# MPEGGroup/mpeg-pcc-tmc2

Measured on AMD Instinct MI355X. Metric: encoder patch+image-gen frames/sec, longdress_vox10 32-frame GOF, higher is better.
Workload: dtype int32/f64

## Files before the change

mpeg-pcc-tmc2_amd/csrc/kdtree_device.hip:

```cpp
#include <algorithm>
#include <cstring>

#include "internal.h"
#include "wave.h"

namespace tmc2 {
namespace {

constexpr uint32_t kNone      = 0xFFFFFFFFu;
constexpr int      kBlock     = 256;
constexpr int      kWaves     = kBlock / 64;
constexpr int      kScanTile  = kBlock * 8;
constexpr int      kLeafMax   = 10;
constexpr int      kMaxLevels = 64;

struct BuildSeg {
  uint32_t begin, end;
  uint32_t node, parent;
  int32_t  mn[3], mx[3];
  int16_t  lo[3], hi[3];
  uint8_t  side, pdim;
  uint8_t  split, cutDim;
  int32_t  cut;
  uint32_t mid;
  uint32_t slot;
};

struct RetiredSeg {
  uint32_t begin, end, node, level;
  int16_t  lo[3], hi[3];
  int32_t  root;
};

struct HugeSeg {
  uint32_t begin, end, node, level;
  int16_t  lo[3], hi[3];
  int32_t  root;
  int32_t  mn[3], mx[3];
};

struct BuildArgs {
  const Pt* pts;
  uint32_t  n, tiles;
  Pt*       P;
  uint32_t *perm, *seg;
  BuildSeg *segA, *segB;
  KdNode*   nodes;
  uint32_t *loc1, *loc2, *tile1, *tile2;
  uint32_t* counts;
  uint32_t* nodeCount;
  int32_t*  rootBox;
  uint32_t* levels;
  RetiredSeg* retired;
  uint32_t*   retiredCount;
  uint32_t*   bigCount;
  HugeSeg*    huge;
  uint32_t*   hugeCount;
  uint32_t    hugeMax;
  uint32_t    retireMax, splitMax;
  struct LvSeg *lvA, *lvB;
  uint16_t*   list;
  struct LvPartial* partial;
  unsigned long long* pieceProfile;
  uint32_t    decideRng;
  uint32_t*   finishDepth;
  uint32_t*   ticket;
  volatile uint32_t* hostSmall;
  volatile uint32_t* hostDepth;
};

__device__ __forceinline__ int coordOf( const Pt p, int d ) { return d == 0 ? p.x : ( d == 1 ? p.y : p.z ); }

struct SplitRule {
  int     dim;
  int32_t cut;
};
__device__ __forceinline__ SplitRule splitOf( const int16_t ( &lo )[3], const int16_t ( &hi )[3], const int32_t ( &mn )[3],
                                              const int32_t ( &mx )[3] ) {
  const int32_t maxSpan = max( int32_t( hi[0] ) - lo[0], max( int32_t( hi[1] ) - lo[1], int32_t( hi[2] ) - lo[2] ) );
  SplitRule     r;
  r.dim              = 0;
  int32_t bestSpread = -1;
#pragma unroll
  for ( int d = 0; d < 3; ++d ) {
    if ( double( int32_t( hi[d] ) - lo[d] ) > ( 1.0 - 0.00001 ) * double( maxSpan ) ) {
      const int32_t spread = mx[d] - mn[d];
      if ( spread > bestSpread ) {
        bestSpread = spread;
        r.dim      = d;
      }
    }
  }
  const int32_t l = r.dim == 0 ? lo[0] : ( r.dim == 1 ? lo[1] : lo[2] ), h = r.dim == 0 ? hi[0] : ( r.dim == 1 ? hi[1] : hi[2] );
  const int32_t a = r.dim == 0 ? mn[0] : ( r.dim == 1 ? mn[1] : mn[2] ), b = r.dim == 0 ? mx[0] : ( r.dim == 1 ? mx[1] : mx[2] );
  r.cut           = min( max( ( l + h ) / 2, a ), b );
  return r;
}

constexpr int      kHugeWaves = 16;
constexpr uint32_t kHugeLimit = 131072;
constexpr int      kHugeNodes = 2 * int( kHugeLimit / 4096 ) + 4;
struct HugeNode {
  uint32_t begin, end;
  uint32_t node;
  int16_t  lo[3], hi[3];
  int16_t  mn[3], mx[3];
  uint16_t depth;
};

__device__ __forceinline__ uint32_t blockClassLists( const Pt* pts, uint32_t count, int dim, int32_t c, uint32_t* listGE,
                                                     uint32_t* listLT, uint32_t* waveCnt ) {
  const int lane = threadIdx.x & 63, wave = threadIdx.x >> 6;
  uint32_t  mGE = 0, mIn = 0;
  int       buf = 0;
  for ( uint32_t base = 0; base < count; base += 4u * blockDim.x, buf ^= 1 ) {
    const uint32_t i0 = base + 4u * threadIdx.x;
    bool           ge[4];
    uint32_t       cGE = 0, cIn = 0;
#pragma unroll
    for ( int j = 0; j < 4; ++j ) {
      const bool    in = i0 + j < count;
      const int32_t x  = coordOf( pts[in ? i0 + j : 0u], dim );
      ge[j]            = in && x >= c;
      cGE += uint32_t( ge[j] ), cIn += uint32_t( in );
    }
    const uint32_t inc = waveInclusive( cGE | ( cIn << 16 ), lane );
    if ( lane == 63 ) waveCnt[buf * kHugeWaves + wave] = inc;
    __syncthreads();
    uint32_t before = 0, total = 0;
#pragma unroll
    for ( int w = 0; w < kHugeWaves; ++w ) {
      const uint32_t cw = waveCnt[buf * kHugeWaves + w];
      total += cw;
      before += w < wave ? cw : 0u;
    }
    before += inc - ( cGE | ( cIn << 16 ) );
    uint32_t atGE = mGE + ( before & 0xFFFFu ) + 0u, atIn = mIn + ( before >> 16 );
#pragma unroll
    for ( int j = 0; j < 4; ++j ) {
      if ( i0 + j < count ) {
        if ( ge[j] )
          listGE[atGE] = i0 + j;
        else
          listLT[atIn - atGE] = i0 + j;
        atGE += uint32_t( ge[j] ), ++atIn;
      }
    }
    mGE += total & 0xFFFFu, mIn += total >> 16;
  }
  return mGE;
}

__device__ __forceinline__ uint32_t blockSweep( Pt* pts, uint32_t* id, uint32_t count, int dim, int32_t c, uint32_t* listGE,
                                                uint32_t* listLT, uint32_t* waveCnt ) {
  const uint32_t nGE = blockClassLists( pts, count, dim, c, listGE, listLT, waveCnt ), nL = count - nGE;
  __syncthreads();
  for ( uint32_t t = threadIdx.x; t < min( nGE, nL ); t += blockDim.x ) {
    const uint32_t x = listGE[t];
    if ( x >= nL ) break;
    const uint32_t y  = listLT[nL - 1u - t];
    const Pt       px = pts[x], py = pts[y];
    const uint32_t ix = id[x], iy = id[y];
    pts[x] = py, pts[y] = px, id[x] = iy, id[y] = ix;
  }
  __syncthreads();
  return nL;
}

__global__ __launch_bounds__( 64 * kHugeWaves ) void hugeSegmentsKernel( BuildArgs a ) {
  __shared__ HugeNode sNode[2][kHugeNodes];
  __shared__ uint32_t sCount[2], waveCnt[2 * kHugeWaves];
  __shared__ int32_t  red[kHugeWaves][12];
  const int      lane = threadIdx.x & 63, wave = threadIdx.x >> 6;
  const uint32_t total = *a.hugeCount;
  for ( uint32_t s = blockIdx.x; s < total; s += gridDim.x ) {
    const HugeSeg seg = a.huge[s];
    __syncthreads();
    if ( threadIdx.x == 0 ) {
      HugeNode r;
      r.begin = 0, r.end = seg.end - seg.begin, r.node = seg.node, r.depth = 0;
      for ( int d = 0; d < 3; ++d ) r.lo[d] = seg.lo[d], r.hi[d] = seg.hi[d], r.mn[d] = int16_t( seg.mn[d] ), r.mx[d] = int16_t( seg.mx[d] );
      sNode[0][0] = r;
      sCount[0] = 1, sCount[1] = 0;
    }
    __syncthreads();
    int cur = 0;
    for ( uint32_t depth = 0;; ++depth ) {
      const uint32_t nCur = sCount[cur];
      if ( nCur == 0 ) break;
      for ( uint32_t t = 0; t < nCur; ++t ) {
        const HugeNode q     = sNode[cur][t];
        const uint32_t count = q.end - q.begin;
        if ( uint32_t( q.depth ) + seg.level >= uint32_t( kMaxLevels ) - 2u ) {
          if ( threadIdx.x == 0 ) atomicMax( a.finishDepth, 0x10000u );
          continue;
        }
        Pt*       pts = a.P + seg.begin + q.begin;
        uint32_t* id  = a.perm + seg.begin + q.begin;
        int32_t   mn[3], mx[3];
        const bool isRoot = seg.root != 0 && depth == 0;
        int16_t    lo[3], hi[3];
        for ( int d = 0; d < 3; ++d ) mn[d] = q.mn[d], mx[d] = q.mx[d], lo[d] = isRoot ? q.mn[d] : q.lo[d], hi[d] = isRoot ? q.mx[d] : q.hi[d];
        const SplitRule rule  = splitOf( lo, hi, mn, mx );
        uint32_t*       listA = a.loc1 + seg.begin + q.begin;
        uint32_t*       listB = a.loc2 + seg.begin + q.begin;
        const uint32_t  lt    = blockSweep( pts, id, count, rule.dim, rule.cut, listA, listB, waveCnt );
        const uint32_t  le    = lt + blockSweep( pts + lt, id + lt, count - lt, rule.dim, rule.cut + 1, listA, listB, waveCnt );
        const uint32_t  half  = count / 2;
        const uint32_t  idx   = lt > half ? lt : ( le < half ? le : half );
        int32_t r[12];
#pragma unroll
        for ( int k = 0; k < 12; ++k ) r[k] = ( k % 6 ) < 3 ? 0x7FFFFFFF : int32_t( 0x80000000 );
        for ( uint32_t base = 0; base < count; base += 4u * blockDim.x ) {
          Pt p[4];
#pragma unroll
          for ( int j = 0; j < 4; ++j ) {
            const uint32_t i = base + j * blockDim.x + threadIdx.x;
            p[j]             = pts[i < count ? i : 0u];
          }
#pragma unroll
          for ( int j = 0; j < 4; ++j ) {
            const uint32_t i = base + j * blockDim.x + threadIdx.x;
            if ( i < count ) {
              const int o = i < idx ? 0 : 6;
              if ( o == 0 ) {
                r[0] = min( r[0], int32_t( p[j].x ) ), r[1] = min( r[1], int32_t( p[j].y ) ), r[2] = min( r[2], int32_t( p[j].z ) );
                r[3] = max( r[3], int32_t( p[j].x ) ), r[4] = max( r[4], int32_t( p[j].y ) ), r[5] = max( r[5], int32_t( p[j].z ) );
              } else {
                r[6] = min( r[6], int32_t( p[j].x ) ), r[7] = min( r[7], int32_t( p[j].y ) ), r[8] = min( r[8], int32_t( p[j].z ) );
                r[9] = max( r[9], int32_t( p[j].x ) ), r[10] = max( r[10], int32_t( p[j].y ) ), r[11] = max( r[11], int32_t( p[j].z ) );
              }
            }
          }
        }
#pragma unroll
        for ( int off = 32; off > 0; off >>= 1 )
#pragma unroll
          for ( int k = 0; k < 12; ++k ) {
            const int32_t o = __shfl_xor( r[k], off, 64 );
            r[k]            = ( k % 6 ) < 3 ? min( r[k], o ) : max( r[k], o );
          }
        if ( lane == 0 )
          for ( int k = 0; k < 12; ++k ) red[wave][k] = r[k];
        __syncthreads();
        if ( threadIdx.x == 0 ) {
          for ( int w = 0; w < kHugeWaves; ++w )
            for ( int k = 0; k < 12; ++k ) r[k] = ( k % 6 ) < 3 ? min( r[k], red[w][k] ) : max( r[k], red[w][k] );
          const uint32_t id0 = atomicAdd( a.nodeCount, 2u );
          KdNode         nd;
          nd.a = int32_t( id0 ), nd.b = int32_t( id0 + 1 ), nd.divlow = int16_t( r[3 + rule.dim] ), nd.divhigh = int16_t( r[6 + rule.dim] ),
          nd.dim = rule.dim;
          a.nodes[q.node] = nd;
          HugeNode child[2];
          child[0].begin = q.begin, child[0].end = q.begin + idx, child[0].node = id0;
          child[1].begin = q.begin + idx, child[1].end = q.end, child[1].node = id0 + 1;
          for ( int c = 0; c < 2; ++c ) {
            child[c].depth = uint16_t( q.depth + 1 );
            for ( int d = 0; d < 3; ++d )
              child[c].lo[d] = lo[d], child[c].hi[d] = hi[d], child[c].mn[d] = int16_t( r[6 * c + d] ), child[c].mx[d] = int16_t( r[6 * c + 3 + d] );
          }
          const int16_t cut = int16_t( rule.cut );
          if ( rule.dim == 0 ) child[0].hi[0] = cut, child[1].lo[0] = cut;
          if ( rule.dim == 1 ) child[0].hi[1] = cut, child[1].lo[1] = cut;
          if ( rule.dim == 2 ) child[0].hi[2] = cut, child[1].lo[2] = cut;
          for ( int c = 0; c < 2; ++c ) {
            const uint32_t cc = child[c].end - child[c].begin, level = seg.level + child[c].depth;
            if ( cc <= uint32_t( kLeafMax ) ) {
              KdNode leaf;
              leaf.a = int32_t( seg.begin + child[c].begin ), leaf.b = int32_t( seg.begin + child[c].end ), leaf.divlow = leaf.divhigh = 0,
              leaf.dim = -1;
              a.nodes[child[c].node] = leaf;
              atomicMax( a.finishDepth, level + 1u );
            } else if ( cc <= a.retireMax ) {
              RetiredSeg rs;
              rs.begin = seg.begin + child[c].begin, rs.end = seg.begin + child[c].end, rs.node = child[c].node, rs.level = level, rs.root = 0;
              for ( int d = 0; d < 3; ++d ) rs.lo[d] = child[c].lo[d], rs.hi[d] = child[c].hi[d];
              a.retired[atomicAdd( a.retiredCount, 1u )] = rs;
            } else {
              sNode[cur ^ 1][sCount[cur ^ 1]++] = child[c];
            }
          }
        }
        __syncthreads();
      }
      if ( threadIdx.x == 0 ) sCount[cur] = 0;
      cur ^= 1;
      __syncthreads();
    }
  }
}

constexpr int      kPieceMax  = 4096;
constexpr int      kPieceRecs = kPieceMax / ( kLeafMax + 1 ) + 2;
constexpr uint16_t kNoRec     = 0xFFFFu;
constexpr uint32_t kNoKey     = 0xFFFFFFFFu;

struct alignas( 8 ) PieceRec {
  uint16_t begin, end;
  int16_t  cut;
  uint8_t  dim, unused0;
// ... 15 lines not shown
  uint32_t e1rb1, e2rb2;
};
struct PieceHot2 {
  uint32_t midc0, c1;
};

__device__ __forceinline__ void pieceBarrier() { asm volatile( "s_waitcnt lgkmcnt(0)\n\ts_barrier" ::: "memory" ); }

typedef short pkShort2 __attribute__( ( ext_vector_type( 2 ) ) );
__device__ __forceinline__ uint32_t pkMin( uint32_t a, uint32_t b ) {
  return __builtin_bit_cast( uint32_t, __builtin_elementwise_min( __builtin_bit_cast( pkShort2, a ), __builtin_bit_cast( pkShort2, b ) ) );
}
__device__ __forceinline__ uint32_t pkMax( uint32_t a, uint32_t b ) {
  return __builtin_bit_cast( uint32_t, __builtin_elementwise_max( __builtin_bit_cast( pkShort2, a ), __builtin_bit_cast( pkShort2, b ) ) );
}
__device__ __forceinline__ uint32_t pk2( int lo16, int hi16 ) { return ( uint32_t( lo16 ) & 0xFFFFu ) | ( uint32_t( hi16 ) << 16 ); }
__device__ __forceinline__ int      pkLo( uint32_t v ) { return int( int16_t( v & 0xFFFFu ) ); }
__device__ __forceinline__ int      pkHi( uint32_t v ) { return int( int16_t( v >> 16 ) ); }

template <int WAVES>
__device__ __forceinline__ uint32_t pieceScan( uint32_t v, uint32_t* waveTot ) {
  const int lane = threadIdx.x & 63, wave = threadIdx.x >> 6;
  const uint32_t inc = waveInclusive( v, lane );
  if ( lane == 63 ) waveTot[wave] = inc;
  pieceBarrier();
  uint32_t before = 0;
#pragma unroll
  for ( int w = 0; w < WAVES; w += 4 ) {
    const uint4 t = *reinterpret_cast<const uint4*>( waveTot + w );
    before += ( w + 0 < wave ? t.x : 0u ) + ( w + 1 < wave ? t.y : 0u ) + ( w + 2 < wave ? t.z : 0u ) + ( w + 3 < wave ? t.w : 0u );
  }
  return before + inc - v;
}

__device__ __forceinline__ bool waveSegMinMaxPacked( uint32_t key, uint32_t& A, uint32_t& B, uint32_t& C, int lane ) {
#pragma unroll
  for ( int off = 1; off < 64; off <<= 1 ) {
    const uint32_t ok = __shfl_down( key, off, 64 );
    const uint32_t oa = __shfl_down( A, off, 64 ), ob = __shfl_down( B, off, 64 ), oc = __shfl_down( C, off, 64 );
    if ( lane + off < 64 && ok == key ) A = pkMin( A, oa ), B = pkMax( B, ob ), C = pkMin( C, oc );
  }
  const uint32_t pk = __shfl_up( key, 1, 64 );
  return key != kNoKey && ( lane == 0 || pk != key );
}

__device__ __forceinline__ void ldsMin( int32_t* slot, int32_t v ) {
  if ( v < *reinterpret_cast<volatile int32_t*>( slot ) ) atomicMin( slot, v );
}
__device__ __forceinline__ void ldsMax( int32_t* slot, int32_t v ) {
  if ( v > *reinterpret_cast<volatile int32_t*>( slot ) ) atomicMax( slot, v );
}


struct LvSeg {
  uint32_t begin, end;
  uint32_t cutInfo;
  uint32_t edge1;
  uint32_t slot;
  uint32_t childNode;
  uint32_t node, parent;
  int16_t  lo[3], hi[3];
  uint8_t  side, pdim;
  uint16_t unused;
  int32_t  mn[3], mx[3];
};

constexpr int kLandBlock = 256;
constexpr int kLandRounds = 2;
struct LvPartial {
  uint32_t slot;
  uint32_t v[6];
  uint32_t unused;
};

__device__ __forceinline__ void lvReport( LvSeg* child, int mnx, int mny, int mnz, int mxx, int mxy, int mxz ) {
  if ( mnx < loadStaleOk( &child->mn[0] ) ) atomicMin( &child->mn[0], mnx );
  if ( mny < loadStaleOk( &child->mn[1] ) ) atomicMin( &child->mn[1], mny );
  if ( mnz < loadStaleOk( &child->mn[2] ) ) atomicMin( &child->mn[2], mnz );
  if ( mxx > loadStaleOk( &child->mx[0] ) ) atomicMax( &child->mx[0], mxx );
  if ( mxy > loadStaleOk( &child->mx[1] ) ) atomicMax( &child->mx[1], mxy );
  if ( mxz > loadStaleOk( &child->mx[2] ) ) atomicMax( &child->mx[2], mxz );
}

__device__ __forceinline__ uint32_t lvPrefix( const uint32_t* __restrict__ loc, const uint32_t* sums, uint32_t tiles, uint32_t i, uint32_t n ) {
  return i < n ? loc[i] + sums[i / kScanTile] : sums[tiles];
}

__device__ __forceinline__ uint32_t lvPartner( const uint16_t* __restrict__ list, const uint32_t* sums, uint32_t from, uint32_t to, uint32_t G ) {
  uint32_t lo = from / kScanTile, hi = ( to - 1u ) / kScanTile;
  while ( lo < hi ) {
    const uint32_t mid = ( lo + hi + 1u ) / 2u;
    if ( mid * kScanTile - sums[mid] <= G )
      lo = mid;
    else
      hi = mid - 1u;
  }
  return lo * kScanTile + list[size_t( lo ) * kScanTile + ( G - ( lo * kScanTile - sums[lo] ) )];
}

__global__ __launch_bounds__( kBlock ) void lvInitKernel( BuildArgs a ) {
  __shared__ int blockRange[6 * kWaves];
  const uint32_t n = a.n, gsize = gridDim.x * blockDim.x;
  const int      lane = threadIdx.x & 63, wave = threadIdx.x >> 6;
  int mnx = 0x7FFFFFFF, mny = mnx, mnz = mnx, mxx = int( 0x80000000 ), mxy = mxx, mxz = mxx;
  for ( uint32_t i = blockIdx.x * blockDim.x + threadIdx.x; i < n; i += gsize ) {
    const Pt p = a.pts[i];
    a.P[i]     = p;
    a.perm[i]  = i;
    a.seg[i]   = 0;
    mnx = min( mnx, int( p.x ) ), mny = min( mny, int( p.y ) ), mnz = min( mnz, int( p.z ) );
    mxx = max( mxx, int( p.x ) ), mxy = max( mxy, int( p.y ) ), mxz = max( mxz, int( p.z ) );
  }
  mnx = waveMin( mnx ), mny = waveMin( mny ), mnz = waveMin( mnz );
  mxx = waveMax( mxx ), mxy = waveMax( mxy ), mxz = waveMax( mxz );
  if ( lane == 0 ) {
    int* w = blockRange + 6 * wave;
    w[0] = mnx, w[1] = mny, w[2] = mnz, w[3] = mxx, w[4] = mxy, w[5] = mxz;
  }
  __syncthreads();
  if ( threadIdx.x < 6 ) {
    int v = blockRange[threadIdx.x];
    for ( int w = 1; w < kWaves; ++w ) v = threadIdx.x < 3 ? min( v, blockRange[6 * w + threadIdx.x] ) : max( v, blockRange[6 * w + threadIdx.x] );
    int32_t* slot = threadIdx.x < 3 ? &a.lvA[0].mn[threadIdx.x] : &a.lvA[0].mx[threadIdx.x - 3];
    if ( threadIdx.x < 3 ) {
      if ( v < loadStaleOk( slot ) ) atomicMin( slot, v );
    } else {
      if ( v > loadStaleOk( slot ) ) atomicMax( slot, v );
    }
  }
}
__global__ void lvRootKernel( BuildArgs a ) {
  if ( threadIdx.x < kMaxLevels + 16 ) a.counts[threadIdx.x] = 0;
  __syncthreads();
  if ( threadIdx.x != 0 ) return;
  LvSeg r{};
  r.begin = 0, r.end = a.n, r.node = 0, r.parent = kNone;
  for ( int d = 0; d < 3; ++d ) r.mn[d] = 0x7FFFFFFF, r.mx[d] = int32_t( 0x80000000 );
  a.lvA[0]     = r;
// ... 85 lines not shown
        const int32_t maxSpan = max( hi[0] - lo[0], max( hi[1] - lo[1], hi[2] - lo[2] ) );
        const double  limit   = ( 1.0 - 0.00001 ) * double( maxSpan );
        int           dim     = 0;
        int32_t       best    = -1;
        if ( double( hi[0] - lo[0] ) > limit && mx[0] - mn[0] > best ) best = mx[0] - mn[0], dim = 0;
        if ( double( hi[1] - lo[1] ) > limit && mx[1] - mn[1] > best ) best = mx[1] - mn[1], dim = 1;
        if ( double( hi[2] - lo[2] ) > limit && mx[2] - mn[2] > best ) best = mx[2] - mn[2], dim = 2;
        const int32_t l = dim == 0 ? lo[0] : ( dim == 1 ? lo[1] : lo[2] ), h = dim == 0 ? hi[0] : ( dim == 1 ? hi[1] : hi[2] );
        const int32_t lowest = dim == 0 ? mn[0] : ( dim == 1 ? mn[1] : mn[2] ), highest = dim == 0 ? mx[0] : ( dim == 1 ? mx[1] : mx[2] );
        const int32_t cut = min( max( ( l + h ) / 2, lowest ), highest );
        q->cutInfo = ( uint32_t( cut ) & 0xFFFFu ) | ( uint32_t( dim ) << 16 ) | ( 1u << 24 );
        if ( root )
          for ( int d = 0; d < 3; ++d ) q->lo[d] = int16_t( mn[d] ), q->hi[d] = int16_t( mx[d] );
        split = 1;
      }
      if ( !split ) q->cutInfo = 0;
    }
    const uint32_t inc = waveInclusive( split, lane );
    if ( lane == 63 ) waveTot[wave] = inc;
    __syncthreads();
    uint32_t before = sCarry, all = 0;
    for ( int w = 0; w < kDecideThreads / 64; ++w ) {
      all += waveTot[w];
      before += w < wave ? waveTot[w] : 0u;
    }
    const uint32_t rank = before + inc - split;
    if ( split ) q->slot = 2u * rank, q->childNode = nodeBase + 2u * rank;
    __syncthreads();
    if ( threadIdx.x == 0 ) sCarry += all;
    __syncthreads();
  }
  if ( threadIdx.x == 0 ) {
    a.counts[level + 1] = 2u * sCarry;
    *a.nodeCount        = nodeBase + 2u * sCarry;
  }
  if ( a.hostSmall ) {
    if ( threadIdx.x == 0 ) __threadfence();
    __syncthreads();
    if ( threadIdx.x < kMaxLevels + 16 ) a.hostSmall[threadIdx.x] = __hip_atomic_load( &a.counts[threadIdx.x], __ATOMIC_RELAXED, __HIP_MEMORY_SCOPE_AGENT );
  }
}

template <bool FIRST>
__global__ __launch_bounds__( kBlock ) void lvFlagKernel( BuildArgs a, uint32_t level ) {
  __shared__ uint32_t waveTot[kWaves];
  const uint32_t n = a.n, tiles = a.tiles;
  LvSeg*         cur   = ( level & 1 ) ? a.lvB : a.lvA;
  LvSeg*         next  = ( level & 1 ) ? a.lvA : a.lvB;
  const uint32_t count = a.counts[level];
  uint32_t*      loc   = FIRST ? a.loc1 : a.loc2;
  uint32_t*      tile  = FIRST ? a.tile1 : a.tile2;
  if ( !FIRST ) {
    for ( uint32_t s = blockIdx.x * blockDim.x + threadIdx.x; s < count; s += gridDim.x * blockDim.x ) {
      const LvSeg* q = cur + s;
      if ( !( q->cutInfo >> 24 ) ) continue;
      for ( int c = 0; c < 2; ++c )
        for ( int d = 0; d < 3; ++d ) next[q->slot + c].mn[d] = 0x7FFFFFFF, next[q->slot + c].mx[d] = int32_t( 0x80000000 );
    }
  }
  for ( uint32_t t = blockIdx.x; t < tiles; t += gridDim.x ) {
    const uint32_t base = t * kScanTile + threadIdx.x * 8;
    uint32_t       v[8], run = 0;
#pragma unroll
    for ( int k = 0; k < 8; ++k ) {
      const uint32_t i = base + k;
      uint32_t       f = 0;
      if ( i < n ) {
        const uint32_t s = a.seg[i];
        if ( s != kNone ) {
          const LvSeg*   q  = cur + s;
          const uint32_t ci = q->cutInfo;
          if ( ci >> 24 ) {
            const int32_t c = int32_t( int16_t( ci & 0xFFFFu ) ), x = coordOf( a.P[i], int( ( ci >> 16 ) & 0xFFu ) );
            f               = FIRST ? uint32_t( x >= c ) : uint32_t( i >= q->edge1 && x > c );
          }
        }
      }
      v[k] = f;
      run += f;
    }
    uint32_t offset = blockExclusive<kWaves>( run, waveTot );
#pragma unroll
    for ( int k = 0; k < 8; ++k ) {
      if ( base + k < n ) {
        loc[base + k] = offset;
        if ( !v[k] ) a.list[size_t( t ) * kScanTile + ( threadIdx.x * 8 + k - offset )] = uint16_t( threadIdx.x * 8 + k );
      }
      offset += v[k];
    }
    if ( threadIdx.x == kBlock - 1 ) tile[t] = offset;
    __syncthreads();
  }
}

template <int BLOCK>
__device__ __forceinline__ void lvLoadSums( uint32_t* sums, const uint32_t* __restrict__ raw, uint32_t tiles ) {
  __shared__ uint32_t waveTot[BLOCK / 64];
  uint32_t            carry = 0;
  for ( uint32_t base = 0; base < tiles; base += BLOCK ) {
    const uint32_t i   = base + threadIdx.x;
    const uint32_t v   = i < tiles ? raw[i] : 0u;
    uint32_t       all;
    const uint32_t offset = carry + blockExclusive<BLOCK / 64>( v, waveTot, all );
    if ( i < tiles ) sums[i] = offset;
    carry += all;
    __syncthreads();
  }
  if ( threadIdx.x == 0 ) sums[tiles] = carry;
  __syncthreads();
}

__global__ __launch_bounds__( kBlock ) void lvSwapOneKernel( BuildArgs a, uint32_t level ) {
  extern __shared__ uint32_t lvSums[];
  const uint32_t n = a.n, tiles = a.tiles;
  const uint32_t gsize = gridDim.x * blockDim.x;
  LvSeg*         cur = ( level & 1 ) ? a.lvB : a.lvA;
  lvLoadSums<kBlock>( lvSums, a.tile1, tiles );
  for ( uint32_t i = blockIdx.x * blockDim.x + threadIdx.x; i < n; i += gsize ) {
    const uint32_t s = a.seg[i];
    if ( s == kNone ) continue;
    LvSeg*         q  = cur + s;
    const uint32_t ci = q->cutInfo;
    if ( !( ci >> 24 ) ) continue;
    const uint32_t b = q->begin, e = q->end;
    const Pt       pi = a.P[i];
    const uint32_t li = a.loc1[i];
    const uint32_t rb = lvPrefix( a.loc1, lvSums, tiles, b, n ), re = lvPrefix( a.loc1, lvSums, tiles, e, n );
    const uint32_t edge = b + ( ( e - b ) - ( re - rb ) );
    if ( i == b ) q->edge1 = edge;
    if ( i >= edge || coordOf( pi, int( ( ci >> 16 ) & 0xFFu ) ) < int32_t( int16_t( ci & 0xFFFFu ) ) ) continue;
    const uint32_t r  = li + lvSums[i / kScanTile] - rb;
    const uint32_t j  = lvPartner( a.list, lvSums, edge, e, ( e - re ) - 1u - r );
    const Pt       pj = a.P[j];
    a.P[i]            = pj;
    a.P[j]            = pi;
    const uint32_t u  = a.perm[i];
    a.perm[i]         = a.perm[j];
    a.perm[j]         = u;
  }
}

__global__ __launch_bounds__( kLandBlock ) void lvSwapTwoKernel( BuildArgs a, uint32_t level ) {
  extern __shared__ uint32_t lvSums[];
  const uint32_t n = a.n, tiles = a.tiles;
  const int      lane  = threadIdx.x & 63;
  LvSeg*         cur  = ( level & 1 ) ? a.lvB : a.lvA;
  LvSeg*         next = ( level & 1 ) ? a.lvA : a.lvB;
  lvLoadSums<kLandBlock>( lvSums, a.tile2, tiles );
  const uint32_t nRound = ( n + uint32_t( kLandBlock ) - 1u ) & ~( uint32_t( kLandBlock ) - 1u );
  __shared__ uint32_t blockSeg;
  __shared__ uint32_t red[kLandBlock / 64][6];
  __shared__ uint32_t accV[6], accSlot;
  const int wave = threadIdx.x >> 6;
  constexpr uint32_t kChunk = uint32_t( kLandBlock ) * kLandRounds;
  for ( uint32_t c0 = blockIdx.x * kChunk; c0 < nRound; c0 += gridDim.x * kChunk ) {
  if ( threadIdx.x == 0 ) accSlot = kNone;
  for ( uint32_t i0 = c0; i0 < min( c0 + kChunk, nRound ); i0 += kLandBlock ) {
    const uint32_t i   = i0 + threadIdx.x;
    uint32_t       key = kNoKey;
    uint32_t       A = pk2( 0x7FFF, 0x7FFF ), B = pk2( -0x8000, -0x8000 ), C = pk2( 0x7FFF, 0x7FFF );
    uint32_t       A2 = A, B2 = B, C2 = C;
    bool           moved = false;
    uint32_t       s = kNone, slot = 0;
    if ( i < n ) {
      s           = a.seg[i];
      uint32_t to = kNone;
      if ( s != kNone ) {
        LvSeg*         q  = cur + s;
        const uint32_t ci = q->cutInfo;
        if ( ci >> 24 ) {
          const uint32_t b = q->begin, e = q->end, e1 = q->edge1;
          slot               = q->slot;
          const int      dim = int( ( ci >> 16 ) & 0xFFu );
          const int32_t  cut = int32_t( int16_t( ci & 0xFFFFu ) );
          Pt             pi  = a.P[i];
          const uint32_t li  = a.loc2[i];
          const uint32_t rb = lvPrefix( a.loc2, lvSums, tiles, e1, n ), re = lvPrefix( a.loc2, lvSums, tiles, e, n );
          const uint32_t e2   = e1 + ( ( e - e1 ) - ( re - rb ) );
          const uint32_t cnt  = e - b, half = cnt / 2, lim1 = e1 - b, lim2 = e2 - b;
          const uint32_t idx  = lim1 > half ? lim1 : ( lim2 < half ? lim2 : half );
          const uint32_t mid  = b + idx;
          if ( i == b ) {
            KdNode nd;
            nd.a = int32_t( q->childNode ), nd.b = int32_t( q->childNode + 1u ), nd.divlow = nd.divhigh = 0, nd.dim = dim;
            a.nodes[q->node] = nd;
            for ( int c = 0; c < 2; ++c ) {
              LvSeg* ch = next + slot + c;
              ch->begin = c ? mid : b, ch->end = c ? e : mid, ch->cutInfo = 0, ch->edge1 = 0, ch->slot = 0, ch->childNode = 0;
              ch->node = q->childNode + c, ch->parent = q->node, ch->side = uint8_t( c ), ch->pdim = uint8_t( dim ), ch->unused = 0;
              for ( int d = 0; d < 3; ++d ) ch->lo[d] = q->lo[d], ch->hi[d] = q->hi[d];
              if ( c == 0 ) {
                if ( dim == 0 ) ch->hi[0] = int16_t( cut );
                if ( dim == 1 ) ch->hi[1] = int16_t( cut );
                if ( dim == 2 ) ch->hi[2] = int16_t( cut );
              } else {
                if ( dim == 0 ) ch->lo[0] = int16_t( cut );
                if ( dim == 1 ) ch->lo[1] = int16_t( cut );
                if ( dim == 2 ) ch->lo[2] = int16_t( cut );
              }
            }
          }
          const int32_t x = coordOf( pi, dim );
          to              = slot + ( i >= mid ? 1u : 0u );
          key             = to;
          if ( i >= e1 && i < e2 && x > cut ) {
            const uint32_t r  = li + lvSums[i / kScanTile] - rb;
            const uint32_t j  = lvPartner( a.list, lvSums, e2, e, ( e - re ) - 1u - r );
            const Pt       pj = a.P[j];
            a.P[i]            = pj;
            a.P[j]            = pi;
            const uint32_t u  = a.perm[i];
            a.perm[i]         = a.perm[j];
            a.perm[j]         = u;
            moved             = true;
            A2 = pk2( pi.x, pi.y ), B2 = A2, C2 = pk2( pi.z, ~int( pi.z ) );
            pi = pj;
          }
          if ( !( i >= e2 && x <= cut ) ) A = pk2( pi.x, pi.y ), B = A, C = pk2( pi.z, ~int( pi.z ) );
        }
        a.seg[i] = to;
      }
    }
    if ( threadIdx.x == 0 ) blockSeg = s;
    __syncthreads();
    const bool uniform = __syncthreads_and( s == blockSeg ) != 0;
    if ( uniform ) {
      const bool anything = __syncthreads_or( key != kNoKey ) != 0;
      if ( anything ) {
        uint32_t v[6];
        const bool right = key != kNoKey && key != slot;
        v[0] = right || key == kNoKey ? pk2( 0x7FFF, 0x7FFF ) : A, v[1] = right || key == kNoKey ? pk2( -0x8000, -0x8000 ) : B,
        v[2] = right || key == kNoKey ? pk2( 0x7FFF, 0x7FFF ) : C;
        v[3] = pkMin( right ? A : pk2( 0x7FFF, 0x7FFF ), A2 ), v[4] = pkMax( right ? B : pk2( -0x8000, -0x8000 ), B2 ),
        v[5] = pkMin( right ? C : pk2( 0x7FFF, 0x7FFF ), C2 );
#pragma unroll
        for ( int k = 0; k < 6; ++k ) v[k] = ( k % 3 ) == 1 ? waveReduce( v[k], pkMax ) : waveReduce( v[k], pkMin );
        if ( lane == 0 )
          for ( int k = 0; k < 6; ++k ) red[wave][k] = v[k];
        __syncthreads();
        if ( threadIdx.x == 0 ) {
          uint32_t x[6];
          for ( int k = 0; k < 6; ++k ) {
            x[k] = red[0][k];
            for ( int w = 1; w < kLandBlock / 64; ++w ) x[k] = ( k % 3 ) == 1 ? pkMax( x[k], red[w][k] ) : pkMin( x[k], red[w][k] );
          }
          if ( accSlot != kNone && accSlot != slot ) {
            for ( int c = 0; c < 2; ++c )
              lvReport( next + accSlot + c, pkLo( accV[3 * c] ), pkHi( accV[3 * c] ), pkLo( accV[3 * c + 2] ), pkLo( accV[3 * c + 1] ), pkHi( accV[3 * c + 1] ),
                        ~pkHi( accV[3 * c + 2] ) );
            accSlot = kNone;
          }
          for ( int k = 0; k < 6; ++k ) accV[k] = accSlot == kNone ? x[k] : ( ( k % 3 ) == 1 ? pkMax( accV[k], x[k] ) : pkMin( accV[k], x[k] ) );
          accSlot = slot;
        }
      }
      __syncthreads();
      continue;
    }
    if ( moved ) lvReport( next + slot + 1u, pkLo( A2 ), pkHi( A2 ), pkLo( C2 ), pkLo( A2 ), pkHi( A2 ), pkLo( C2 ) );
    if ( waveSegMinMaxPacked( key, A, B, C, lane ) )
      lvReport( next + key, pkLo( A ), pkHi( A ), pkLo( C ), pkLo( B ), pkHi( B ), ~pkHi( C ) );
  }
  __syncthreads();
  if ( threadIdx.x == 0 ) {
    LvPartial pt;
    pt.slot = accSlot, pt.unused = 0;
    for ( int k = 0; k < 6; ++k ) pt.v[k] = accV[k];
    a.partial[c0 / kChunk] = pt;
  }
  __syncthreads();
  }
// ... 334 lines not shown
            ldsMin( &ch->mn[0], mnx ), ldsMin( &ch->mn[1], mny ), ldsMin( &ch->mn[2], mnz );
            ldsMax( &ch->mx[0], mxx ), ldsMax( &ch->mx[1], mxy ), ldsMax( &ch->mx[2], mxz );
          }
        }
        *reinterpret_cast<uint2*>( segOf + p0 ) = *reinterpret_cast<const uint2*>( out );
      }
      cur ^= 1;
    }
    if ( deepest ) atomicMax( &sDepth, deepest );
    if ( PROFILE && threadIdx.x == 0 ) {
      for ( int k = 0; k < 8; ++k ) atomicAdd( a.pieceProfile + k, prof[k] ), prof[k] = 0;
      atomicAdd( a.pieceProfile + 8, 1ull );
    }
    pieceBarrier();
    for ( uint32_t i = tid; i < cnt; i += THREADS ) {
      a.P[seg.begin + i]    = P[i];
      a.perm[seg.begin + i] = perm[i];
    }
    if ( tid == 0 && sDepth ) atomicMax( a.finishDepth, sDepth );
  }
  if ( a.hostDepth && tid == 0 ) {
    __threadfence();
    if ( atomicAdd( a.ticket, 1u ) == gridDim.x - 1u ) {
      __threadfence();
      *a.hostDepth = __hip_atomic_load( a.finishDepth, __ATOMIC_RELAXED, __HIP_MEMORY_SCOPE_AGENT );
    }
  }
}

}

int buildKdTreeDevice( tmc2_ctx* ctx, const Pt* d_pts, uint64_t n64, DeviceTree& tree ) {
  const uint32_t n = uint32_t( n64 );
  tree.n           = n64;
  tree.depth       = 0;
  for ( int d = 0; d < 3; ++d ) tree.lo[d] = tree.hi[d] = 0;
  if ( n == 0 ) return TMC2_OK;
  hipStream_t    s       = ctx->stream;
  const uint32_t tiles   = ( n + kScanTile - 1 ) / kScanTile;
  const size_t   maxSegs = 2 * ( size_t( n ) / ( kLeafMax + 1 ) + 1 ) + 2;
  const size_t   maxNode = 2 * size_t( n ) + 2;
  TMC2_TRY( tree.ptsTree.alloc( size_t( n ) + 1 ) );
  TMC2_TRY( tree.perm.alloc( n ) );
  TMC2_TRY( tree.nodes.alloc( maxNode ) );
  DevBuf<uint32_t>   d_work, d_small;
  DevBuf<BuildSeg>   d_segs;
  DevBuf<RetiredSeg> d_retired;
  const size_t       maxRetired = size_t( n ) / ( kLeafMax + 1 ) + 2;
  TMC2_TRY( d_retired.alloc( maxRetired ) );
  DevBuf<HugeSeg> d_huge;
  TMC2_TRY( d_huge.alloc( size_t( n ) / ( kPieceMax + 1 ) + 2 ) );
  const auto     hugeEnv = ctxOption( ctx, "KD_HUGEMAX" );
  const uint32_t hugeMax = std::min<uint32_t>( kHugeLimit, std::max<uint32_t>( kPieceMax, hugeEnv ? uint32_t( atoi( hugeEnv->c_str() ) ) : 16384u ) );
  TMC2_TRY( d_work.alloc( 3 * size_t( n ) + 2 * ( size_t( tiles ) + 1 ) ) );
  TMC2_TRY( d_segs.alloc( 2 * maxSegs ) );
  TMC2_TRY( d_small.alloc( kMaxLevels + 16 ) );
  static_assert( kMaxLevels + 16 <= 128, "lvRootKernel clears the counters with one workgroup of 128" );
  BuildArgs a;
  a.pts = d_pts, a.n = n, a.tiles = tiles, a.P = tree.ptsTree.p, a.perm = tree.perm.p;
  a.seg = d_work.p, a.loc1 = d_work.p + n, a.loc2 = d_work.p + 2 * size_t( n );
  a.tile1 = d_work.p + 3 * size_t( n ), a.tile2 = a.tile1 + tiles + 1;
  a.segA = d_segs.p, a.segB = d_segs.p + maxSegs, a.nodes = tree.nodes.p;
  a.counts    = d_small.p;
  a.nodeCount = d_small.p + kMaxLevels + 1;
  a.levels    = d_small.p + kMaxLevels + 2;
  a.rootBox   = reinterpret_cast<int32_t*>( d_small.p + kMaxLevels + 8 );
  a.retired      = d_retired.p;
  a.retiredCount = d_small.p + kMaxLevels + 3;
  a.finishDepth  = d_small.p + kMaxLevels + 4;
  a.ticket       = d_small.p + kMaxLevels + 5;
  a.bigCount     = d_small.p + kMaxLevels + 6;
  a.huge         = d_huge.p;
  a.hugeCount    = d_small.p + kMaxLevels + 7;
  a.hugeMax      = hugeMax;
  a.hostSmall    = nullptr;
  a.hostDepth    = ctx->answerLine( tmc2_ctx::kAnswerTreeDepth );
  a.retireMax    = uint32_t( kPieceMax );
  a.splitMax     = uint32_t( kPieceMax );
  const dim3 blk( kBlock ), grdE( std::max<uint32_t>( 1u, ( n + 2 * kBlock - 1 ) / ( 2 * kBlock ) ) ), grdT( tiles );
  const dim3 grdL( std::max<uint32_t>( 1u, ( n + kLandBlock * kLandRounds - 1 ) / ( kLandBlock * kLandRounds ) ) );
  const size_t sumsLds = ( size_t( tiles ) + 1 ) * 4;
  if ( sumsLds > 48 * 1024 ) {
    setError( "kdtree: %u points -- the level passes hold one word per 2 048-point tile in LDS (at most 25 M points)", n );
    return TMC2_E_UNSUPPORTED;
  }
  DevBuf<LvSeg>    d_lv;
  DevBuf<uint16_t> d_list;
  DevBuf<LvPartial> d_partial;
  const size_t     maxLv = 2 * ( size_t( n ) / ( size_t( kPieceMax ) + 1 ) + 2 );
  TMC2_TRY( d_lv.alloc( 2 * maxLv ) );
  TMC2_TRY( d_list.alloc( size_t( tiles ) * kScanTile ) );
  TMC2_TRY( d_partial.alloc( size_t( n ) / ( kLandBlock * kLandRounds ) + 2 ) );
  a.lvA = d_lv.p, a.lvB = d_lv.p + maxLv, a.list = d_list.p, a.partial = d_partial.p;
  const auto decideOpt = ctxOption( ctx, "KD_DECIDE" );
  a.decideRng = decideOpt && ( *decideOpt )[0] == 'g' ? 0u : uint32_t( kDecideRng );
  hipLaunchKernelGGL( lvRootKernel, dim3( 1 ), dim3( 128 ), 0, s, a );
  hipLaunchKernelGGL( lvInitKernel, dim3( std::min<uint32_t>( grdE.x, 1024u ) ), blk, 0, s, a );
  hipLaunchKernelGGL( lvDecideKernel, dim3( 1 ), dim3( kDecideThreads ), 0, s, a, 0u );
  uint32_t out[kMaxLevels + 16];
  int      found = -1;
  int& hint = ctx->kdLevelHint[( n >> 15 ) * 2u + 1u];
  for ( uint32_t level = 0; level < uint32_t( kMaxLevels ) && found < 0; ) {
    uint32_t chunkEnd = level + 1;
    if ( level == 0 && hint > 0 ) {
      chunkEnd = uint32_t( std::min( hint, kMaxLevels ) );
    } else {
      while ( chunkEnd < uint32_t( kMaxLevels ) && ( uint64_t( hugeMax ) << std::min<uint32_t>( chunkEnd - 1, 40 ) ) < n ) ++chunkEnd;
      if ( chunkEnd == level + 1 ) chunkEnd = std::min<uint32_t>( level + 2, kMaxLevels );
    }
    volatile uint32_t* hostSmall = ctx->answerLine( tmc2_ctx::kAnswerTreeLevels );
    for ( ; level < chunkEnd; ++level ) {
      hipLaunchKernelGGL( lvFlagKernel<true>, grdT, blk, 0, s, a, level );
      hipLaunchKernelGGL( lvSwapOneKernel, grdE, blk, sumsLds, s, a, level );
      hipLaunchKernelGGL( lvFlagKernel<false>, grdT, blk, 0, s, a, level );
// ... 61 lines not shown
```

Measured before the change: 210.3.

## Vectorize kd-tree build loads and stores and pin loads to batch memory traffic

Reworks the kd-tree build kernels to use 64- and 128-bit vector loads and stores for points, segment ids, scan offsets and the LvSeg records. LvSeg is padded to 80 bytes and 16-byte aligned so a whole row can be read or written at once, and the work arrays are padded to multiples of 8. Empty asm register pins force loads to be issued early so they overlap, and the cross-wave bounding-box reduction is spread over 12 threads instead of one. This cuts the number of memory transactions and serial latency, at the cost of higher register pressure and reliance on the new alignment and padding assumptions.

```diff
diff --git a/mpeg-pcc-tmc2_amd/csrc/kdtree_device.hip b/mpeg-pcc-tmc2_amd/csrc/kdtree_device.hip
--- a/mpeg-pcc-tmc2_amd/csrc/kdtree_device.hip
+++ b/mpeg-pcc-tmc2_amd/csrc/kdtree_device.hip
@@ -71,6 +71,20 @@
 
 __device__ __forceinline__ int coordOf( const Pt p, int d ) { return d == 0 ? p.x : ( d == 1 ? p.y : p.z ); }
 
+typedef uint32_t LvW2 __attribute__( ( ext_vector_type( 2 ) ) );
+typedef uint32_t LvW4 __attribute__( ( ext_vector_type( 4 ) ) );
+__device__ __forceinline__ void lvPin( uint32_t& a ) { asm volatile( "" : "+v"( a ) ); }
+__device__ __forceinline__ void lvPin( LvW2& a ) { asm volatile( "" : "+v"( a ) ); }
+__device__ __forceinline__ void lvPin( LvW4& a ) { asm volatile( "" : "+v"( a ) ); }
+template <typename T, typename... Rest>
+__device__ __forceinline__ void lvPin( T& a, Rest&... rest ) {
+  lvPin( a );
+  lvPin( rest... );
+}
+__device__ __forceinline__ int32_t lvCoord( LvW2 p, int d ) {
+  return d == 0 ? int32_t( int16_t( p.x & 0xFFFFu ) ) : ( d == 1 ? int32_t( int16_t( p.x >> 16 ) ) : int32_t( int16_t( p.y & 0xFFFFu ) ) );
+}
+
 struct SplitRule {
   int     dim;
   int32_t cut;
@@ -117,10 +131,14 @@
     const uint32_t i0 = base + 4u * threadIdx.x;
     bool           ge[4];
     uint32_t       cGE = 0, cIn = 0;
+    LvW2           pw[4];
+#pragma unroll
+    for ( int j = 0; j < 4; ++j ) pw[j] = *reinterpret_cast<const LvW2*>( pts + ( i0 + j < count ? i0 + j : 0u ) );
+    lvPin( pw[0], pw[1], pw[2], pw[3] );
 #pragma unroll
     for ( int j = 0; j < 4; ++j ) {
       const bool    in = i0 + j < count;
-      const int32_t x  = coordOf( pts[in ? i0 + j : 0u], dim );
+      const int32_t x  = lvCoord( pw[j], dim );
       ge[j]            = in && x >= c;
       cGE += uint32_t( ge[j] ), cIn += uint32_t( in );
     }
@@ -156,9 +174,9 @@
   const uint32_t nGE = blockClassLists( pts, count, dim, c, listGE, listLT, waveCnt ), nL = count - nGE;
   __syncthreads();
   for ( uint32_t t = threadIdx.x; t < min( nGE, nL ); t += blockDim.x ) {
-    const uint32_t x = listGE[t];
+    uint32_t x = listGE[t], y = listLT[nL - 1u - t];
+    lvPin( x, y );
     if ( x >= nL ) break;
-    const uint32_t y  = listLT[nL - 1u - t];
     const Pt       px = pts[x], py = pts[y];
     const uint32_t ix = id[x], iy = id[y];
     pts[x] = py, pts[y] = px, id[x] = iy, id[y] = ix;
@@ -243,9 +261,15 @@
         if ( lane == 0 )
           for ( int k = 0; k < 12; ++k ) red[wave][k] = r[k];
         __syncthreads();
+        if ( threadIdx.x < 12 ) {
+          int32_t v = red[0][threadIdx.x];
+          for ( int w = 1; w < kHugeWaves; ++w ) v = ( threadIdx.x % 6 ) < 3 ? min( v, red[w][threadIdx.x] ) : max( v, red[w][threadIdx.x] );
+          red[0][threadIdx.x] = v;
+        }
+        __syncthreads();
         if ( threadIdx.x == 0 ) {
-          for ( int w = 0; w < kHugeWaves; ++w )
-            for ( int k = 0; k < 12; ++k ) r[k] = ( k % 6 ) < 3 ? min( r[k], red[w][k] ) : max( r[k], red[w][k] );
+#pragma unroll
+          for ( int k = 0; k < 12; ++k ) r[k] = red[0][k];
           const uint32_t id0 = atomicAdd( a.nodeCount, 2u );
           KdNode         nd;
           nd.a = int32_t( id0 ), nd.b = int32_t( id0 + 1 ), nd.divlow = int16_t( r[3 + rule.dim] ), nd.divhigh = int16_t( r[6 + rule.dim] ),
@@ -367,7 +391,7 @@
 }
 
 
-struct LvSeg {
+struct alignas( 16 ) LvSeg {
   uint32_t begin, end;
   uint32_t cutInfo;
   uint32_t edge1;
@@ -378,7 +402,12 @@
   uint8_t  side, pdim;
   uint16_t unused;
   int32_t  mn[3], mx[3];
+  uint32_t pad[2];
 };
+static_assert( sizeof( LvSeg ) == 80 && offsetof( LvSeg, slot ) == 16 && offsetof( LvSeg, lo ) == 32 && offsetof( LvSeg, mn ) == 48, "LvSeg rows" );
+
+__device__ __forceinline__ LvW4 lvRow( const LvSeg* q, int row ) { return reinterpret_cast<const LvW4*>( q )[row]; }
+__device__ __forceinline__ void lvStoreRow( LvSeg* q, int row, LvW4 w ) { reinterpret_cast<LvW4*>( q )[row] = w; }
 
 constexpr int kLandBlock = 256;
 constexpr int kLandRounds = 2;
@@ -389,16 +418,26 @@
 };
 
 __device__ __forceinline__ void lvReport( LvSeg* child, int mnx, int mny, int mnz, int mxx, int mxy, int mxz ) {
-  if ( mnx < loadStaleOk( &child->mn[0] ) ) atomicMin( &child->mn[0], mnx );
-  if ( mny < loadStaleOk( &child->mn[1] ) ) atomicMin( &child->mn[1], mny );
-  if ( mnz < loadStaleOk( &child->mn[2] ) ) atomicMin( &child->mn[2], mnz );
-  if ( mxx > loadStaleOk( &child->mx[0] ) ) atomicMax( &child->mx[0], mxx );
-  if ( mxy > loadStaleOk( &child->mx[1] ) ) atomicMax( &child->mx[1], mxy );
-  if ( mxz > loadStaleOk( &child->mx[2] ) ) atomicMax( &child->mx[2], mxz );
+  uint32_t s0 = uint32_t( loadStaleOk( &child->mn[0] ) ), s1 = uint32_t( loadStaleOk( &child->mn[1] ) ), s2 = uint32_t( loadStaleOk( &child->mn[2] ) );
+  uint32_t s3 = uint32_t( loadStaleOk( &child->mx[0] ) ), s4 = uint32_t( loadStaleOk( &child->mx[1] ) ), s5 = uint32_t( loadStaleOk( &child->mx[2] ) );
+  lvPin( s0, s1, s2, s3, s4, s5 );
+  if ( mnx < int32_t( s0 ) ) atomicMin( &child->mn[0], mnx );
+  if ( mny < int32_t( s1 ) ) atomicMin( &child->mn[1], mny );
+  if ( mnz < int32_t( s2 ) ) atomicMin( &child->mn[2], mnz );
+  if ( mxx > int32_t( s3 ) ) atomicMax( &child->mx[0], mxx );
+  if ( mxy > int32_t( s4 ) ) atomicMax( &child->mx[1], mxy );
+  if ( mxz > int32_t( s5 ) ) atomicMax( &child->mx[2], mxz );
 }
 
 __device__ __forceinline__ uint32_t lvPrefix( const uint32_t* __restrict__ loc, const uint32_t* sums, uint32_t tiles, uint32_t i, uint32_t n ) {
   return i < n ? loc[i] + sums[i / kScanTile] : sums[tiles];
+}
+__device__ __forceinline__ void lvPrefix2( const uint32_t* __restrict__ loc, const uint32_t* sums, uint32_t tiles, uint32_t i0, uint32_t i1, uint32_t n,
+                                           uint32_t& r0, uint32_t& r1 ) {
+  uint32_t l0 = loc[min( i0, n - 1u )], l1 = loc[min( i1, n - 1u )];
+  lvPin( l0, l1 );
+  r0 = i0 < n ? l0 + sums[i0 / kScanTile] : sums[tiles];
+  r1 = i1 < n ? l1 + sums[i1 / kScanTile] : sums[tiles];
 }
 
 __device__ __forceinline__ uint32_t lvPartner( const uint16_t* __restrict__ list, const uint32_t* sums, uint32_t from, uint32_t to, uint32_t G ) {
@@ -590,42 +629,67 @@
   uint32_t*      tile  = FIRST ? a.tile1 : a.tile2;
   if ( !FIRST ) {
     for ( uint32_t s = blockIdx.x * blockDim.x + threadIdx.x; s < count; s += gridDim.x * blockDim.x ) {
-      const LvSeg* q = cur + s;
-      if ( !( q->cutInfo >> 24 ) ) continue;
-      for ( int c = 0; c < 2; ++c )
-        for ( int d = 0; d < 3; ++d ) next[q->slot + c].mn[d] = 0x7FFFFFFF, next[q->slot + c].mx[d] = int32_t( 0x80000000 );
+      const LvSeg* q  = cur + s;
+      uint32_t     ci = q->cutInfo, slot = q->slot;
+      lvPin( ci, slot );
+      if ( !( ci >> 24 ) ) continue;
+      for ( int c = 0; c < 2; ++c ) {
+        uint32_t* w = reinterpret_cast<uint32_t*>( next[slot + c].mn );
+        *reinterpret_cast<LvW4*>( w )     = LvW4{0x7FFFFFFFu, 0x7FFFFFFFu, 0x7FFFFFFFu, 0x80000000u};
+        *reinterpret_cast<LvW2*>( w + 4 ) = LvW2{0x80000000u, 0x80000000u};
+      }
     }
   }
   for ( uint32_t t = blockIdx.x; t < tiles; t += gridDim.x ) {
     const uint32_t base = t * kScanTile + threadIdx.x * 8;
-    uint32_t       v[8], run = 0;
+    uint32_t       run = 0, flags = 0, liveAt = 0;
+    LvW4           sA = LvW4{kNone, kNone, kNone, kNone}, sB = sA;
+    if ( base < n ) sA = *reinterpret_cast<const LvW4*>( a.seg + base );
+    if ( base + 4 < n ) sB = *reinterpret_cast<const LvW4*>( a.seg + base + 4 );
+    lvPin( sA, sB );
+    uint32_t sg[8] = {sA.x, sA.y, sA.z, sA.w, sB.x, sB.y, sB.z, sB.w};
+    uint32_t ci[8], e1[8];
+    LvW4     pp[4];
 #pragma unroll
     for ( int k = 0; k < 8; ++k ) {
-      const uint32_t i = base + k;
-      uint32_t       f = 0;
-      if ( i < n ) {
-        const uint32_t s = a.seg[i];
-        if ( s != kNone ) {
-          const LvSeg*   q  = cur + s;
-          const uint32_t ci = q->cutInfo;
-          if ( ci >> 24 ) {
-            const int32_t c = int32_t( int16_t( ci & 0xFFFFu ) ), x = coordOf( a.P[i], int( ( ci >> 16 ) & 0xFFu ) );
-            f               = FIRST ? uint32_t( x >= c ) : uint32_t( i >= q->edge1 && x > c );
-          }
-        }
-      }
-      v[k] = f;
+      if ( base + k >= n ) sg[k] = kNone;
+      liveAt |= uint32_t( sg[k] != kNone ) << k;
+      const LvSeg* q = cur + ( sg[k] != kNone ? sg[k] : 0u );
+      if ( FIRST ) {
+        ci[k] = q->cutInfo, e1[k] = 0;
+      } else {
+        const LvW2 w = *reinterpret_cast<const LvW2*>( &q->cutInfo );
+        ci[k] = w.x, e1[k] = w.y;
+      }
+    }
+#pragma unroll
+    for ( int m = 0; m < 4; ++m ) pp[m] = *reinterpret_cast<const LvW4*>( a.P + ( base + 2 * m < n ? base + 2 * m : 0u ) );
+#pragma unroll
+    for ( int k = 0; k < 8; ++k ) lvPin( ci[k] ), lvPin( e1[k] );
+    lvPin( pp[0], pp[1], pp[2], pp[3] );
+#pragma unroll
+    for ( int k = 0; k < 8; ++k ) {
+      const uint32_t i  = base + k;
+      const uint32_t lw = ( k & 1 ) ? pp[k / 2].z : pp[k / 2].x, hw = ( k & 1 ) ? pp[k / 2].w : pp[k / 2].y;
+      const int      dim = int( ( ci[k] >> 16 ) & 0xFFu );
+      const int32_t  c = int32_t( int16_t( ci[k] & 0xFFFFu ) );
+      const int32_t  x = dim == 0 ? int32_t( int16_t( lw & 0xFFFFu ) ) : ( dim == 1 ? int32_t( int16_t( lw >> 16 ) ) : int32_t( int16_t( hw & 0xFFFFu ) ) );
+      const bool     live = ( ( liveAt >> k ) & 1u ) != 0 && ( ci[k] >> 24 ) != 0;
+      const uint32_t f    = live ? ( FIRST ? uint32_t( x >= c ) : uint32_t( i >= e1[k] && x > c ) ) : 0u;
+      flags |= f << k;
       run += f;
     }
     uint32_t offset = blockExclusive<kWaves>( run, waveTot );
+    uint32_t at[8];
 #pragma unroll
     for ( int k = 0; k < 8; ++k ) {
-      if ( base + k < n ) {
-        loc[base + k] = offset;
-        if ( !v[k] ) a.list[size_t( t ) * kScanTile + ( threadIdx.x * 8 + k - offset )] = uint16_t( threadIdx.x * 8 + k );
-      }
-      offset += v[k];
-    }
+      at[k] = offset;
+      const uint32_t f = ( flags >> k ) & 1u;
+      if ( base + k < n && !f ) a.list[size_t( t ) * kScanTile + ( threadIdx.x * 8 + k - offset )] = uint16_t( threadIdx.x * 8 + k );
+      offset += f;
+    }
+    if ( base < n ) *reinterpret_cast<LvW4*>( loc + base ) = LvW4{at[0], at[1], at[2], at[3]};
+    if ( base + 4 < n ) *reinterpret_cast<LvW4*>( loc + base + 4 ) = LvW4{at[4], at[5], at[6], at[7]};
     if ( threadIdx.x == kBlock - 1 ) tile[t] = offset;
     __syncthreads();
   }
@@ -701,60 +765,64 @@
     bool           moved = false;
     uint32_t       s = kNone, slot = 0;
     if ( i < n ) {
-      s           = a.seg[i];
+      s = a.seg[i];
+      LvW2     pw;
+      uint32_t li, u;
       uint32_t to = kNone;
       if ( s != kNone ) {
-        LvSeg*         q  = cur + s;
-        const uint32_t ci = q->cutInfo;
+        LvSeg* q  = cur + s;
+        LvW4   r0 = lvRow( q, 0 ), r1 = lvRow( q, 1 ), r2 = lvRow( q, 2 );
+        pw = *reinterpret_cast<const LvW2*>( a.P + i ), li = a.loc2[i], u = a.perm[i];
+        lvPin( r0, r1, r2, pw, li, u );
+        const uint32_t ci = r0.z;
         if ( ci >> 24 ) {
-          const uint32_t b = q->begin, e = q->end, e1 = q->edge1;
-          slot               = q->slot;
+          const uint32_t b = r0.x, e = r0.y, e1 = r0.w;
+          slot               = r1.x;
           const int      dim = int( ( ci >> 16 ) & 0xFFu );
           const int32_t  cut = int32_t( int16_t( ci & 0xFFFFu ) );
-          Pt             pi  = a.P[i];
-          const uint32_t li  = a.loc2[i];
-          const uint32_t rb = lvPrefix( a.loc2, lvSums, tiles, e1, n ), re = lvPrefix( a.loc2, lvSums, tiles, e, n );
+          uint32_t       rb, re;
+          lvPrefix2( a.loc2, lvSums, tiles, e1, e, n, rb, re );
           const uint32_t e2   = e1 + ( ( e - e1 ) - ( re - rb ) );
           const uint32_t cnt  = e - b, half = cnt / 2, lim1 = e1 - b, lim2 = e2 - b;
           const uint32_t idx  = lim1 > half ? lim1 : ( lim2 < half ? lim2 : half );
           const uint32_t mid  = b + idx;
           if ( i == b ) {
-            KdNode nd;
-            nd.a = int32_t( q->childNode ), nd.b = int32_t( q->childNode + 1u ), nd.divlow = nd.divhigh = 0, nd.dim = dim;
-            a.nodes[q->node] = nd;
-            for ( int c = 0; c < 2; ++c ) {
-              LvSeg* ch = next + slot + c;
-              ch->begin = c ? mid : b, ch->end = c ? e : mid, ch->cutInfo = 0, ch->edge1 = 0, ch->slot = 0, ch->childNode = 0;
-              ch->node = q->childNode + c, ch->parent = q->node, ch->side = uint8_t( c ), ch->pdim = uint8_t( dim ), ch->unused = 0;
-              for ( int d = 0; d < 3; ++d ) ch->lo[d] = q->lo[d], ch->hi[d] = q->hi[d];
-              if ( c == 0 ) {
-                if ( dim == 0 ) ch->hi[0] = int16_t( cut );
-                if ( dim == 1 ) ch->hi[1] = int16_t( cut );
-                if ( dim == 2 ) ch->hi[2] = int16_t( cut );
-              } else {
-                if ( dim == 0 ) ch->lo[0] = int16_t( cut );
-                if ( dim == 1 ) ch->lo[1] = int16_t( cut );
-                if ( dim == 2 ) ch->lo[2] = int16_t( cut );
-              }
-            }
+            const uint32_t childNode = r1.y, node = r1.z;
+            KdNode         nd;
+            nd.a = int32_t( childNode ), nd.b = int32_t( childNode + 1u ), nd.divlow = nd.divhigh = 0, nd.dim = dim;
+            a.nodes[node] = nd;
+            const uint32_t c16 = uint32_t( cut ) & 0xFFFFu;
+            LvW4           left = r2, right = r2;
+            if ( dim == 0 ) left.y = ( r2.y & 0x0000FFFFu ) | ( c16 << 16 ), right.x = ( r2.x & 0xFFFF0000u ) | c16;
+            if ( dim == 1 ) left.z = ( r2.z & 0xFFFF0000u ) | c16, right.x = ( r2.x & 0x0000FFFFu ) | ( c16 << 16 );
+            if ( dim == 2 ) left.z = ( r2.z & 0x0000FFFFu ) | ( c16 << 16 ), right.y = ( r2.y & 0xFFFF0000u ) | c16;
+            left.w = uint32_t( dim ) << 8, right.w = 1u | ( uint32_t( dim ) << 8 );
+            LvSeg* ch = next + slot;
+            lvStoreRow( ch, 0, LvW4{b, mid, 0u, 0u} );
+            lvStoreRow( ch, 1, LvW4{0u, 0u, childNode, node} );
+            lvStoreRow( ch, 2, left );
+            lvStoreRow( ch + 1, 0, LvW4{mid, e, 0u, 0u} );
+            lvStoreRow( ch + 1, 1, LvW4{0u, 0u, childNode + 1u, node} );
+            lvStoreRow( ch + 1, 2, right );
           }
-          const int32_t x = coordOf( pi, dim );
+          const int32_t x = lvCoord( pw, dim );
           to              = slot + ( i >= mid ? 1u : 0u );
           key             = to;
           if ( i >= e1 && i < e2 && x > cut ) {
             const uint32_t r  = li + lvSums[i / kScanTile] - rb;
             const uint32_t j  = lvPartner( a.list, lvSums, e2, e, ( e - re ) - 1u - r );
-            const Pt       pj = a.P[j];
-            a.P[i]            = pj;
-            a.P[j]            = pi;
-            const uint32_t u  = a.perm[i];
-            a.perm[i]         = a.perm[j];
-            a.perm[j]         = u;
-            moved             = true;
-            A2 = pk2( pi.x, pi.y ), B2 = A2, C2 = pk2( pi.z, ~int( pi.z ) );
-            pi = pj;
+            LvW2           pj = *reinterpret_cast<const LvW2*>( a.P + j );
+            uint32_t       uj = a.perm[j];
+            lvPin( pj, uj );
+            *reinterpret_cast<LvW2*>( a.P + i ) = pj;
+            *reinterpret_cast<LvW2*>( a.P + j ) = pw;
+            a.perm[i]                            = uj;
+            a.perm[j]                            = u;
+            moved                                = true;
+            A2 = pw.x, B2 = A2, C2 = pk2( lvCoord( pw, 2 ), ~lvCoord( pw, 2 ) );
+            pw = pj;
           }
-          if ( !( i >= e2 && x <= cut ) ) A = pk2( pi.x, pi.y ), B = A, C = pk2( pi.z, ~int( pi.z ) );
+          if ( !( i >= e2 && x <= cut ) ) A = pw.x, B = A, C = pk2( lvCoord( pw, 2 ), ~lvCoord( pw, 2 ) );
         }
         a.seg[i] = to;
       }
@@ -1195,14 +1263,15 @@
   TMC2_TRY( d_huge.alloc( size_t( n ) / ( kPieceMax + 1 ) + 2 ) );
   const auto     hugeEnv = ctxOption( ctx, "KD_HUGEMAX" );
   const uint32_t hugeMax = std::min<uint32_t>( kHugeLimit, std::max<uint32_t>( kPieceMax, hugeEnv ? uint32_t( atoi( hugeEnv->c_str() ) ) : 16384u ) );
-  TMC2_TRY( d_work.alloc( 3 * size_t( n ) + 2 * ( size_t( tiles ) + 1 ) ) );
+  const size_t nPad = ( size_t( n ) + 7 ) & ~size_t( 7 );
+  TMC2_TRY( d_work.alloc( 3 * nPad + 2 * ( size_t( tiles ) + 1 ) ) );
   TMC2_TRY( d_segs.alloc( 2 * maxSegs ) );
   TMC2_TRY( d_small.alloc( kMaxLevels + 16 ) );
   static_assert( kMaxLevels + 16 <= 128, "lvRootKernel clears the counters with one workgroup of 128" );
   BuildArgs a;
   a.pts = d_pts, a.n = n, a.tiles = tiles, a.P = tree.ptsTree.p, a.perm = tree.perm.p;
-  a.seg = d_work.p, a.loc1 = d_work.p + n, a.loc2 = d_work.p + 2 * size_t( n );
-  a.tile1 = d_work.p + 3 * size_t( n ), a.tile2 = a.tile1 + tiles + 1;
+  a.seg = d_work.p, a.loc1 = d_work.p + nPad, a.loc2 = d_work.p + 2 * nPad;
+  a.tile1 = d_work.p + 3 * nPad, a.tile2 = a.tile1 + tiles + 1;
   a.segA = d_segs.p, a.segB = d_segs.p + maxSegs, a.nodes = tree.nodes.p;
   a.counts    = d_small.p;
   a.nodeCount = d_small.p + kMaxLevels + 1;
```

New measurement: 218.9, median of 6. 4.1% higher.
